# gisbi-kim/navtech-radar-slam

Measured on AMD Instinct MI355X. Metric: sc_loop_queries_per_sec_vs_10k_scan_db, higher is better.
Workload: dtype f16 filter + f64 exact

## Files before the change

navtech-radar-slam_amd/csrc/sc_api.cpp:

```cpp
#include <cmath>
#include <cstdio>
#include <cstdlib>
#include <cstring>
#include <mutex>
#include <new>
#include <string>
#include <vector>

#include "rsx_common.h"
#include "sc_kernels.h"
#include "sc_plan.h"
#include "sc_kdtree.h"
#include "loopverify.h"
#include "radarsc.h"
#include "voxelgrid.h"

namespace rsx {
std::string &last_error() {
  static thread_local std::string e;
  return e;
}
}

using namespace rsx;
// ... 1530 lines not shown
int rsx_sc_merge_topk(const rsx_sc_hit *parts, int32_t nparts, int32_t nq, int32_t k, rsx_sc_hit *out) try {
  if (!parts || !out || nparts < 1 || nq < 1 || k < 1) return fail(RSX_ERR_BAD_ARG, "bad arg");
  for (int q = 0; q < nq; q++) {
    rsx_sc_hit *o = out + (size_t)q * k;
    int count = 0;
    for (int p = 0; p < nparts; p++)
      for (int i = 0; i < k; i++) {
        const rsx_sc_hit &r = parts[((size_t)p * nq + q) * k + i];
        if (!(r.dist < 10000000)) continue;
        int pos = count < k ? count : k;
        while (pos > 0 && ((r.dist < o[pos - 1].dist) || (r.dist == o[pos - 1].dist && r.index < o[pos - 1].index))) pos--;
        if (pos >= k) continue;
        int last = count < k ? count : k - 1;
        for (int j = last; j > pos; j--) o[j] = o[j - 1];
        o[pos] = r;
        if (count < k) count++;
      }
    for (int i = count; i < k; i++) {
      o[i].dist = 10000000;
      o[i].index = 0;
      o[i].shift = 0;
    }
  }
  return RSX_OK;
} RSX_CATCH_ALL

int rsx_sc_merge_topk_device(rsx_sc *h, const rsx_sc_hit *d_parts, int32_t nparts, int32_t nq, int32_t k,
                             rsx_sc_hit *d_out, void *stream) try {
  if (!h || !d_parts || !d_out || nparts < 1 || nq < 1 || k < 1 || k > RSX_SC_MAX_TOPK) return fail(RSX_ERR_BAD_ARG, "bad arg");
  std::lock_guard<std::mutex> lk(h->mu);
  RSX_TRY(set_device(h));
  hipStream_t s;
  RSX_TRY(use_stream(h, stream, &s));
  return launch_merge(d_parts, nparts, nq, k, d_out, s);
} RSX_CATCH_ALL

int rsx_sc_profile_enable(rsx_sc *h, int on) try {
  if (!h) return fail(RSX_ERR_BAD_ARG, "null handle");
  std::lock_guard<std::mutex> lk(h->mu);
  RSX_TRY(own_stream(h));
  if (on && !h->prof.ev) {
    h->prof.ev.reset(new (std::nothrow) Event[2 * PairProfiler::kMax]);
    if (!h->prof.ev) return fail(RSX_ERR_OOM, "host alloc");
    for (int i = 0; i < 2 * PairProfiler::kMax; i++) RSX_HIP(h->prof.ev[i].create(true));
  }
  if (on) {
    RSX_TRY(h->stats.reserve(kStatBytes, h->stream, false));
    RSX_HIP(hipMemsetAsync(h->stats.p, 0, kStatBytes, h->stream));
    RSX_HIP(hipStreamSynchronize(h->stream));
  }
  h->prof.on = on != 0;
  h->prof.used = 0;
  return RSX_OK;
} RSX_CATCH_ALL

int rsx_sc_profile_read_rescoring(rsx_sc *h, rsx_sc_rescoring_stats *out) try {
  if (!h || !out || out->struct_size < offsetof(rsx_sc_rescoring_stats, candidates)) return fail(RSX_ERR_BAD_ARG, "null arg / struct_size not set");
  int64_t out6[8];
  int64_t *const out5 = out6;
  int64_t *candidates = out5, *exact_evals = out5 + 1, *queries_rescored = out5 + 2;
  struct Publish {
    rsx_sc_rescoring_stats *o;
    const int64_t *v;
    ~Publish() {
      int64_t *dst = &o->candidates;
      const size_t n = (o->struct_size - offsetof(rsx_sc_rescoring_stats, candidates)) / sizeof(int64_t);
      for (size_t i = 0; i < n && i < 8; i++) dst[i] = v[i];
    }
  } publish{out, out6};
  std::lock_guard<std::mutex> lk(h->mu);
  RSX_TRY(set_device(h));
  for (int i = 0; i < 8; i++) out6[i] = 0;
  if (!h->stats.p) return RSX_OK;
  RSX_HIP(hipDeviceSynchronize());
  unsigned long long v[RESCORE_STAT_WORDS] = {0};
  {
    std::vector<unsigned long long> all((size_t)RESCORE_STAT_COPIES * RESCORE_STAT_WORDS);
    RSX_HIP(hipMemcpy(all.data(), h->stats.p, kStatBytes, hipMemcpyDeviceToHost));
    RSX_HIP(hipMemset(h->stats.p, 0, kStatBytes));
    for (int c = 0; c < RESCORE_STAT_COPIES; c++)
      for (int i = 0; i < RESCORE_STAT_WORDS; i++) v[i] += all[(size_t)c * RESCORE_STAT_WORDS + i];
  }
  if (rsx::exp_env("RSX_RESCORE_PROF") && v[1])
    fprintf(stderr, "[sc_rescore prof] per query (cycles): start loads %.0f  round filter + touch %.0f  pick %.0f  phaseB %.0f  align %.0f  entry wait %.0f  total %.0f\n",
            (double)v[4] / v[1], (double)v[5] / v[1], (double)v[6] / v[1], (double)v[7] / v[1], (double)v[8] / v[1], (double)v[9] / v[1],
            (double)v[10] / v[1]);
  *candidates = (int64_t)v[0];
  *exact_evals = v[2] ? (int64_t)v[2] : (int64_t)v[0];
  *queries_rescored = (int64_t)v[1];
  out5[3] = (int64_t)v[3];
  out5[4] = (int64_t)v[11];
  out6[5] = v[12] ? (int64_t)v[12] : 7 * *exact_evals;
  out6[6] = (int64_t)v[15];
  out6[7] = (int64_t)v[16];
  return RSX_OK;
} RSX_CATCH_ALL

int rsx_sc_profile_read(rsx_sc *h, int64_t *launches, double *total_ms) try {
  if (!h || !launches || !total_ms) return fail(RSX_ERR_BAD_ARG, "null arg");
  std::lock_guard<std::mutex> lk(h->mu);
  RSX_TRY(set_device(h));
  *launches = 0;
  *total_ms = 0.0;
  for (int i = 0; i < h->prof.used; i++) {
    RSX_HIP(hipEventSynchronize(h->prof.ev[2 * i + 1]));
    float ms = 0.f;
    RSX_HIP(hipEventElapsedTime(&ms, h->prof.ev[2 * i], h->prof.ev[2 * i + 1]));
    *total_ms += ms;
    (*launches)++;
  }
  h->prof.used = 0;
  return RSX_OK;
} RSX_CATCH_ALL

int rsx_sc_hit_to_loop(rsx_sc *h, const rsx_sc_hit *hit, int32_t *loop_id, float *yaw) try {
  if (!h || !hit) return fail(RSX_ERR_BAD_ARG, "null arg");
  std::lock_guard<std::mutex> lk(h->mu);
  if (loop_id) *loop_id = (hit->dist < h->p.dist_thres) ? hit->index : -1;
  if (yaw) *yaw = yaw_from_shift(hit->shift);
  return RSX_OK;
} RSX_CATCH_ALL

}
```

navtech-radar-slam_amd/csrc/sc_exact_dev.h:

```cpp
#pragma once
#include <hip/hip_runtime.h>

#include <cmath>
#include <cstdint>

#include "sc_kernels.h"
#include "sc_entry_dev.h"

namespace rsx {
namespace sc {
namespace {

constexpr double kBig = 10000000.0;

constexpr int ENT_VKEY_A = 0, ENT_VKEY_B = 1152, ENT_SIM = 0, ENT_MISC = 3360;
constexpr int ENT_SIZE = 3408;

__device__ __forceinline__ bool hit_before(double ad, int ai, double bd, int bi) {
  return (ad < bd) || (ad == bd && ai < bi);
}

struct EntryRegs {
  float4 ecol[5];
  double v, n2;
};
__device__ __forceinline__ void load_entry(const DbView &db, int64_t slot, int lane, EntryRegs &r) {
  const int cl = lane < NS ? lane : 0;
  r.v = db.vkey[slot * NS + cl];
  const float4 *src = reinterpret_cast<const float4 *>(db.desc + slot * DS + cl * NR);
#pragma unroll
  for (int i = 0; i < 5; i++) r.ecol[i] = src[i];
  r.n2 = db.norm[slot * NS + cl];
}

struct Touch {
  int d0 = 0, d1 = 0, d2 = 0;
};
__device__ __forceinline__ void touch_entry(const DbView &db, int64_t slot, int lane, Touch &t) {
  const int cl = lane < NS ? lane : 0;
  const float *pd = db.desc + slot * DS + cl * NR;
  const double *pk = db.vkey + slot * NS + cl, *pn = db.norm + slot * NS + cl;
  asm volatile("global_load_dword %0, %3, off\n\tglobal_load_dword %1, %4, off\n\tglobal_load_dword %2, %5, off"
               : "+v"(t.d0), "+v"(t.d1), "+v"(t.d2)
               : "v"(pd), "v"(pk), "v"(pn)
               : "memory");
}
__device__ __forceinline__ void touch_keep(Touch &t) { asm volatile("" : "+v"(t.d0), "+v"(t.d1), "+v"(t.d2)); }
__device__ __forceinline__ void touch_wait(Touch &t) {
  asm volatile("s_waitcnt vmcnt(0)" : "+v"(t.d0), "+v"(t.d1), "+v"(t.d2)::"memory");
}

template <int SO = dev::SO_SSE2>
__device__ __forceinline__ int align_exact(const double *v1, char *wsm, int lane, double ev) {
  const int kk = lane < NS ? lane : NS - 1;
  double *vka = reinterpret_cast<double *>(wsm + ENT_VKEY_A);
  double *vkb = reinterpret_cast<double *>(wsm + ENT_VKEY_B);
  if (lane < NS) {
    vka[lane] = ev;
    vka[lane + NS] = ev;
    vkb[lane + 1] = ev;
    vkb[lane + NS + 1] = ev;
  }
  wave::lds_fence();
  double acc[4] = {0.0, 0.0, 0.0, 0.0};
  const int eoff = (kk & 1) ? (ENT_VKEY_B + (NS + 1 - kk) * 8) : (ENT_VKEY_A + (NS - kk) * 8);
  const double2 *v2 = reinterpret_cast<const double2 *>(wsm + eoff);
  const double2 *v1p = reinterpret_cast<const double2 *>(v1);
#pragma unroll 1
  for (int c0 = 0; c0 < NS / 2; c0 += 6) {
#pragma unroll
    for (int cc = 0; cc < 6; cc++) {
      const double2 x = v1p[c0 + cc], y = v2[c0 + cc];
      const double d0 = x.x - y.x;
      const double dd0 = d0 * d0;
      acc[2 * (cc & 1)] = acc[2 * (cc & 1)] + dd0;
      const double d1 = x.y - y.y;
      const double dd1 = d1 * d1;
      acc[2 * (cc & 1) + 1] = acc[2 * (cc & 1) + 1] + dd1;
    }
  }
  double nrm = sqrt((acc[0] + acc[2]) + (acc[1] + acc[3]));
  if constexpr (SO != dev::SO_SSE2) {
    const double *v1d = v1, *v2d = reinterpret_cast<const double *>(wsm + eoff);
    auto d = [&](int c) { return v1d[c] - v2d[c]; };
    nrm = sqrt(dev::redux_prod<SO, NS>(d, d));
  }
  const bool ok = (lane < NS) && (nrm < kBig);
  double m = ok ? nrm : INFINITY;
  m = wave::butterfly(m, [](double a, double b) { return fmin(a, b); });
  const unsigned long long bal = __ballot(ok && nrm == m);
  wave::lds_fence();
  return bal ? (__ffsll((long long)bal) - 1) : 0;
}

__device__ __forceinline__ void topk_insert(double &ld, int &li, int &ls, int lane, int k, double dist, int idx,
                                            int shift) {
  const bool before = (lane < k) && hit_before(ld, li, dist, idx);
  const int pos = __popcll(__ballot(before));
  if (pos < k) {
    double ud = __shfl_up(ld, 1);
    int ui = __shfl_up(li, 1), us = __shfl_up(ls, 1);
    if (lane > pos) {
      ld = ud; li = ui; ls = us;
    } else if (lane == pos) {
      ld = dist; li = idx; ls = shift;
    }
  }
}

__device__ __forceinline__ void topk_insert_dpp(double &ld, int &li, int &ls, int lane, int k, double dist, int idx, int shift) {
  const bool before = (lane < k) && hit_before(ld, li, dist, idx);
  const int pos = __popcll(__ballot(before));
  if (pos < k) {
    const double ud = wave::dpp<0x138>(ld);
    const int ui = wave::dpp<0x138>(li), us = wave::dpp<0x138>(ls);
    if (lane > pos) {
      ld = ud; li = ui; ls = us;
    } else if (lane == pos) {
      ld = dist; li = idx; ls = shift;
    }
  }
}

struct WaveLds {
  static constexpr int OFF_QF32 = 0;
  static constexpr int OFF_QN1 = DS * 4;
  static constexpr int OFF_QV1 = OFF_QN1 + 512;
  static constexpr int OFF_ENT = OFF_QV1 + 512;
  static constexpr int SIZE = OFF_ENT + ENT_SIZE;
};

template <int SO = dev::SO_SSE2>
__device__ __forceinline__ void phase_b32(const char *smem, char *wsm, int lane, const EntryRegs &er, int ks, unsigned tmask,
                                          double &bd_out, int &bk_out) {
  const int cl = lane < NS ? lane : 0;
  const double *qn1 = reinterpret_cast<const double *>(smem + WaveLds::OFF_QN1);
  wave::lds_fence();
  double e[NR];
#pragma unroll
  for (int i = 0; i < 5; i++) {
    const float4 v = er.ecol[i];
    e[4 * i + 0] = v.x; e[4 * i + 1] = v.y; e[4 * i + 2] = v.z; e[4 * i + 3] = v.w;
  }
  const double n2 = er.n2;
  double *simp = reinterpret_cast<double *>(wsm + ENT_SIM);
  int *misc = reinterpret_cast<int *>(wsm + ENT_MISC);
#pragma unroll
  for (int t = 0; t < 7; t++) {
    if (!((tmask >> t) & 1u)) continue;
    int k = ks + t - 3;
    k += (k < 0) ? NS : 0;
    k -= (k >= NS) ? NS : 0;
    int c = cl + k;
    c -= (c >= NS) ? NS : 0;
    const float4 *qp = reinterpret_cast<const float4 *>(smem + WaveLds::OFF_QF32 + c * (NR * 4));
    double da[4] = {0.0, 0.0, 0.0, 0.0};
#pragma unroll
    for (int i = 0; i < 5; i++) {
      const float4 q4 = qp[i];
      da[0] = fma((double)q4.x, e[4 * i + 0], da[0]);
      da[1] = fma((double)q4.y, e[4 * i + 1], da[1]);
      da[2] = fma((double)q4.z, e[4 * i + 2], da[2]);
      da[3] = fma((double)q4.w, e[4 * i + 3], da[3]);
    }
    double dot = (da[0] + da[2]) + (da[1] + da[3]);
    if constexpr (SO != dev::SO_SSE2) {
      const float *qf = reinterpret_cast<const float *>(qp);
      dot = dev::redux_prod<SO, NR>([&](int r) { return (double)qf[r]; }, [&](int r) { return e[r]; });
    }
    const double n1 = qn1[c];
    const bool valid = (lane < NS) && !((n1 == 0.0) | (n2 == 0.0));
    const double s = dot / (n1 * n2);
    if (lane < NS) simp[t * NS + c] = valid ? s : 0.0;
    const int ne = __popcll(__ballot(valid));
    if (lane == 0) misc[t] = ne;
  }
  wave::lds_fence();
  const int tt = lane & 7;
  double bd = INFINITY;
  int bk = 0x7fffffff;
  if (lane < 8 && tt < 7 && ((tmask >> tt) & 1u)) {
    const double2 *sp = reinterpret_cast<const double2 *>(wsm + ENT_SIM + tt * (NS * 8));
    double s = 0.0;
#pragma unroll 1
    for (int c0 = 0; c0 < NS / 2; c0 += 6) {
#pragma unroll
      for (int cc = 0; cc < 6; cc++) {
        const double2 v = sp[c0 + cc];
        s = s + v.x;
        s = s + v.y;
      }
    }
    const int ne = misc[tt];
    const double d = 1.0 - s / (double)ne;
    int k = ks + tt - 3;
    k += (k < 0) ? NS : 0;
    k -= (k >= NS) ? NS : 0;
    if (d < kBig) {
      bd = d;
      bk = k;
    }
  }
#pragma unroll
  for (int off = 1; off <= 4; off <<= 1) {
    const double od = __shfl_xor(bd, off);
    const int ok = __shfl_xor(bk, off);
    if (hit_before(od, ok, bd, bk)) {
      bd = od;
      bk = ok;
    }
  }
  bd = __shfl(bd, 0);
  bk = __shfl(bk, 0);
  if (bd == INFINITY) {
    bd = kBig;
    bk = 0;
  }
  bd_out = bd;
  bk_out = bk;
}

}
}
}
```

navtech-radar-slam_amd/csrc/sc_filter.hip:

```cpp
#include <hip/hip_runtime.h>

#include <cmath>
#include <cstdint>
#include <cstdlib>
#include <type_traits>
#include <utility>

#include "rsx_common.h"
#include "sc_kernels.h"
#include "sc_entry_dev.h"

namespace rsx {
namespace sc {

namespace {

typedef _Float16 half8 __attribute__((ext_vector_type(8)));
typedef float floatx16 __attribute__((ext_vector_type(16)));
typedef unsigned frag4 __attribute__((ext_vector_type(4)));
typedef unsigned long long u64;

#define AS1 __attribute__((address_space(1)))
#define AS3 __attribute__((address_space(3)))

// ... 255 lines not shown
    const int64_t n = tile * 32 + col;
    const bool n_ok = tile_ok && n < a.n_items;
    const int nphase = (q1 - q0 + F_QPP - 1) / F_QPP;

    {
      const int nqs = (q1 - q0 < F_QPP) ? (q1 - q0) : F_QPP;
      stage_queries(a.qimg + (int64_t)q0 * FILTER_QIMG_BYTES, smem, nqs * FILTER_QIMG_BYTES, wave, lane);
    }

    half8 B[F_STEPS];
    {
      const uint4 *src = a.hnT + ((tile_ok ? tile : 0) * F_STEPS) * 64 + lane;
#pragma unroll
      for (int s = 0; s < F_STEPS; s++) {
        const uint4 v = src[s * 64];
        B[s] = *reinterpret_cast<const half8 *>(&v);
      }
#pragma unroll
      for (int s = F_B_VGPR; s < F_STEPS; s++) asm volatile("" : "+a"(B[s]));
    }
    const u64 m2 = n_ok ? a.cmask[n] : 0ull;
    const unsigned m2lo = (unsigned)m2, m2hi = (unsigned)(m2 >> 32) & 0x0fffffffu;

    asm volatile("s_waitcnt vmcnt(0)" ::: "memory");
    __syncthreads();

    floatx16 acc0, acc1, p0;
    frag4 first[F_DEPTH];
    int prev_q = -1;
    u64 prev_mask = 0;
    auto fin = [&](const Epi &ep) {
      float best = epi_end(ep);
      if ((prev_mask | m2) & kNonFinite) best = -INFINITY;
      if (n_ok && hh == 0) a.lb[(int64_t)prev_q * a.ld_lb + n] = lb_pack(best);
    };
    for (int p = 0; p < nphase; p++) {
      const int qp = q0 + p * F_QPP;
      if (p + 1 < nphase) {
        const int qn = qp + F_QPP;
        const int nqs = (q1 - qn < F_QPP) ? (q1 - qn) : F_QPP;
        stage_queries(a.qimg + (int64_t)qn * FILTER_QIMG_BYTES, smem + ((p + 1) & 1) * F_PHASE_BYTES,
                      nqs * FILTER_QIMG_BYTES, wave, lane);
      }
      const int nq_here = (q1 - qp < F_QPP) ? (q1 - qp) : F_QPP;
      if (tile_ok) {
        const unsigned phase_lds = lds_base + (unsigned)((p & 1) * F_PHASE_BYTES + aoff);
        first_prologue(first, phase_lds);
        for (int qq = 0; qq < nq_here; qq++) {
          const unsigned ap_lds = phase_lds + (unsigned)(qq * FILTER_QIMG_BYTES);
          const unsigned next_lds = (qq + 1 < nq_here) ? ap_lds + FILTER_QIMG_BYTES : ap_lds;
          const u64 cur_mask = *reinterpret_cast<const u64 *>(smem + (p & 1) * F_PHASE_BYTES + qq * FILTER_QIMG_BYTES + QIMG_MASK_OFF);
          if (prev_q < 0) filter_stage<true, false>(ap_lds, next_lds, first, B, acc0, acc1, p0, prev_mask, m2lo, m2hi, hh, fin);
          else filter_stage<true, true>(ap_lds, next_lds, first, B, acc0, acc1, p0, prev_mask, m2lo, m2hi, hh, fin);
          prev_q = qp + qq;
          prev_mask = cur_mask;
        }
      }
      asm volatile("s_waitcnt vmcnt(0)" ::: "memory");
      __syncthreads();
    }
    if (prev_q >= 0) filter_stage<false, true>(0u, 0u, first, B, acc0, acc1, p0, prev_mask, m2lo, m2hi, hh, fin);
  }
}

constexpr int H_BINS = RESCORE_BINS;
constexpr int SEL_U = 5;

struct Elig {
  int64_t idx_base, idx_stride, n_eligible;
  const int64_t *q_elig;
};
__device__ __forceinline__ int64_t n_elig_items(const Elig &el, int q, int64_t n_items) {
  int64_t lim = el.n_eligible;
  if (el.q_elig) {
    const int64_t v = el.q_elig[q];
    lim = v < lim ? v : lim;
  }
  if (lim <= el.idx_base) return 0;
  const int64_t c = (lim - el.idx_base + el.idx_stride - 1) / el.idx_stride;
  return c < n_items ? c : n_items;
}


__global__ __launch_bounds__(256) void sc_select_kernel(const lb_t *__restrict__ lb, int64_t ld, int64_t n_items_all,
                                                        Elig el, int32_t first_target,
                                                        RescoreEntry *__restrict__ slist,
                                                        int32_t *__restrict__ sl_cnt, float *__restrict__ thr) {
  __shared__ int hist[H_BINS];
  __shared__ int wsum[4];
  __shared__ int s_bcap;
  __shared__ int s_total;
  const int q = blockIdx.x;
  const int lane = threadIdx.x & 63, wave = threadIdx.x >> 6;
  const lb_t *row = lb + (int64_t)q * ld;
  const int64_t n_items = n_elig_items(el, q, n_items_all);
  for (int i = threadIdx.x; i < H_BINS; i += 256) hist[i] = 0;
  if (threadIdx.x == 0) s_total = 0;
  __syncthreads();
  typedef _Float16 half8 __attribute__((ext_vector_type(8)));
  const uint4 *row8 = reinterpret_cast<const uint4 *>(row);
  const int64_t n8 = n_items >> 3;
  const bool one_piece = n8 <= 256 * SEL_U;
  uint4 keep[SEL_U];
  auto load_piece = [&](int64_t c0, uint4 (&x)[SEL_U]) {
#pragma unroll
    for (int u = 0; u < SEL_U; u++) {
      const int64_t j = c0 + u * 256 + threadIdx.x;
      x[u] = j < n8 ? row8[j] : uint4{0x7c007c00u, 0x7c007c00u, 0x7c007c00u, 0x7c007c00u};
    }
  };
  auto walk_piece = [&](int64_t c0, const uint4 (&x)[SEL_U], auto &&f) {
#pragma unroll
    for (int u = 0; u < SEL_U; u++) {
      const int64_t i = (c0 + u * 256 + threadIdx.x) << 3;
      const half8 h = __builtin_bit_cast(half8, x[u]);
#pragma unroll
      for (int e = 0; e < 8; e++) f((float)h[e], i + e);
    }
  };
  auto for_row = [&](bool first, auto &&f) {
    if (one_piece) {
      if (first) load_piece(0, keep);
      walk_piece(0, keep, f);
    } else {
      for (int64_t c0 = 0; c0 < n8; c0 += 256 * SEL_U) {
        uint4 x[SEL_U];
        load_piece(c0, x);
        walk_piece(c0, x, f);
      }
    }
    const int64_t i = (n8 << 3) + threadIdx.x;
    if (i < n_items) f((float)row[i], i);
  };
  for_row(true, [&](float d, int64_t) {
    if (d != INFINITY) atomicAdd(&hist[lb_bin(d)], 1);
  });
  __syncthreads();
  int v[8];
  int run = 0;
#pragma unroll
  for (int i = 0; i < 8; i++) {
    run += hist[threadIdx.x * 8 + i];
    v[i] = run;
  }
  const int incl = (int)wave::incl_add_u32((unsigned)run);
  if (lane == 63) wsum[wave] = incl;
  __syncthreads();
  int base = incl - run;
  for (int w = 0; w < wave; w++) base += wsum[w];
  __syncthreads();
#pragma unroll
  for (int i = 0; i < 8; i++) hist[threadIdx.x * 8 + i] = base + v[i];
  __syncthreads();
  auto first_reaching = [&](int target) {
    int lo = 0, hi = H_BINS;
    while (lo < hi) {
      const int mid = (lo + hi) >> 1;
      if (hist[mid] >= target) hi = mid;
      else lo = mid + 1;
    }
    return lo;
  };
  if (threadIdx.x == 0) s_bcap = first_reaching(RESCORE_SHORTLIST_CAP + 1) - 1;
  __syncthreads();
  const int b_cap = s_bcap;
  if (threadIdx.x < RESCORE_NUM_THR) {
    int b = b_cap;
    if (threadIdx.x < RESCORE_NUM_THR - 1) {
      b = first_reaching(first_target << threadIdx.x);
      if (b > H_BINS - 1) b = H_BINS - 1;
      if (b > b_cap) b = b_cap;
    }
    thr[(int64_t)q * RESCORE_THR_STRIDE + threadIdx.x] = lb_bin_edge(b);
    reinterpret_cast<int32_t *>(thr)[(int64_t)q * RESCORE_THR_STRIDE + RESCORE_NUM_THR + threadIdx.x] = b >= 0 ? hist[b] : 0;
  }
  int b_head = first_reaching(RESCORE_HEAD);
  if (b_head > b_cap) b_head = b_cap;
  if (threadIdx.x == 0) {
    int32_t *hd = reinterpret_cast<int32_t *>(thr) + (int64_t)q * RESCORE_THR_STRIDE;
    hd[RESCORE_THR_HEAD_BIN] = b_head;
    hd[RESCORE_THR_HEAD_END] = b_head >= 0 ? hist[b_head] : 0;
  }
  RescoreEntry *out = slist + (int64_t)q * RESCORE_SHORTLIST_CAP;
  __shared__ int fill[H_BINS];
  for (int i = threadIdx.x; i < H_BINS; i += 256) fill[i] = i ? hist[i - 1] : 0;
  __syncthreads();
  if (b_head >= 0) {
    for_row(false, [&](float d, int64_t i) {
      if (d == INFINITY) return;
      const int b = lb_bin(d);
      if (b > b_head) return;
      RescoreEntry e;
      e.lb = d;
      e.slot = (int32_t)i;
      out[atomicAdd(&fill[b], 1)] = e;
    });
  }
  if (threadIdx.x == 0) s_total = b_cap >= 0 ? hist[b_cap] : 0;
  __syncthreads();
  if (threadIdx.x == 0) sl_cnt[q] = s_total;
}

__global__ __launch_bounds__(1024) void sc_filter_plan_kernel(Elig el, int32_t nq, int64_t n_items, int32_t qgroup,
                                                              int32_t *__restrict__ tb_qmin, int64_t *__restrict__ tb_cum) {
  __shared__ long long sh[1024];
  const int64_t ntb = (((n_items + 31) >> 5) + 3) >> 2;
  const int t = threadIdx.x;
  long long running = 0;
  for (int64_t base = 0; base < ntb; base += 1024) {
    const int64_t tb = base + t;
    long long items = 0;
    if (tb < ntb) {
      const int64_t g0 = el.idx_base + tb * 128 * el.idx_stride;
      int lo = 0, hi = nq;
      while (lo < hi) {
        const int mid = (lo + hi) >> 1;
        int64_t lim = el.n_eligible;
        if (el.q_elig) {
          const int64_t v = el.q_elig[mid];
          lim = v < lim ? v : lim;
        }
        if (lim > g0) hi = mid;
        else lo = mid + 1;
      }
      tb_qmin[tb] = lo / qgroup;
      items = (nq + qgroup - 1) / qgroup - lo / qgroup;
    }
    sh[t] = items;
    __syncthreads();
    for (int d = 1; d < 1024; d <<= 1) {
      const long long v = t >= d ? sh[t - d] : 0;
      __syncthreads();
      sh[t] += v;
      __syncthreads();
    }
    if (tb < ntb) tb_cum[tb] = running + sh[t] - items;
    running += sh[1023];
    __syncthreads();
  }
  if (t == 0) tb_cum[ntb] = running;
}

}

double filter_eps() {
  static const double eps = [] {
    const char *e = rsx::exp_env("RSX_SC_FILTER_EPS");
    const double v = e ? atof(e) : 0.0;
    return v > 1.25e-3 ? v : 1.25e-3;
  }();
  return eps;
}

size_t filter_qimg_bytes(int32_t nq) { return (size_t)nq * FILTER_QIMG_BYTES + 1024; }

int launch_db_images(const float *desc, const double *norm, int64_t first, int64_t count, void *hnT, void *hnR,
                     uint64_t *cmask, hipStream_t s) {
  if (count <= 0) return RSX_OK;
  hipLaunchKernelGGL(sc_img_db_kernel, dim3((unsigned)((count + 3) / 4)), dim3(256), 0, s, desc, norm, first, count,
                     static_cast<uint4 *>(hnT), static_cast<uint4 *>(hnR), reinterpret_cast<u64 *>(cmask));
  RSX_HIP(hipGetLastError());
  return RSX_OK;
}

int launch_query_images(const float *desc, const double *norm, int32_t nq, void *qimg, hipStream_t s) {
  if (nq <= 0) return RSX_OK;
  hipLaunchKernelGGL(sc_img_query_kernel, dim3((unsigned)((nq + 3) / 4)), dim3(256), 0, s, desc, norm, nq,
                     static_cast<char *>(qimg));
  RSX_HIP(hipGetLastError());
  return RSX_OK;
}

const char *filter_kernel_name() { return "sc_filter_kernel"; }

size_t filter_plan_bytes(int64_t n_items) {
  const int64_t ntb = (((n_items + 31) / 32) + 3) / 4;
  return (size_t)(ntb + 1) * sizeof(int64_t) + (size_t)ntb * sizeof(int32_t) + 64;
}

int launch_filter_plan(const DbView &db, const FilterPlanInput &plan, int32_t nq, int64_t n_items, int32_t qgroup,
                       void *plan_ws, const int32_t **tb_qmin, const int64_t **tb_cum, hipStream_t s) {
  const int64_t ntb = (((n_items + 31) / 32) + 3) / 4;
  int64_t *cum = static_cast<int64_t *>(plan_ws);
  int32_t *qmin = reinterpret_cast<int32_t *>(cum + ntb + 1);
  const Elig el{db.idx_base, db.idx_stride, plan.n_eligible < 0 ? INT64_MAX : plan.n_eligible, plan.q_elig};
  hipLaunchKernelGGL(sc_filter_plan_kernel, dim3(1), dim3(1024), 0, s, el, nq, n_items, qgroup, qmin, cum);
  RSX_HIP(hipGetLastError());
  *tb_qmin = qmin;
  *tb_cum = cum;
  return RSX_OK;
}

int launch_filter(const DbView &db, const void *qimg, int32_t nq, int64_t n_items, lb_t *lb, int64_t ld_lb,
                  const FilterPlanInput *plan, void *plan_ws, hipStream_t s) {
  if (nq <= 0 || n_items <= 0) return RSX_OK;
  static int n_cu = 0;
  const int lds = 2 * F_PHASE_BYTES;
  if (!n_cu) {
    RSX_HIP(hipFuncSetAttribute(reinterpret_cast<const void *>(&sc_filter_kernel),
                                hipFuncAttributeMaxDynamicSharedMemorySize, lds));
    int dev = 0, cu = 0;
    RSX_HIP(hipGetDevice(&dev));
    RSX_HIP(hipDeviceGetAttribute(&cu, hipDeviceAttributeMultiprocessorCount, dev));
    n_cu = cu > 0 ? cu : 256;
  }
  FilterArgs a;
  a.hnT = static_cast<const uint4 *>(db.hnT);
  a.cmask = reinterpret_cast<const u64 *>(db.cmask);
  a.qimg = static_cast<const char *>(qimg);
  a.n_items = n_items;
  a.nq = nq;
  a.lb = lb;
  a.ld_lb = ld_lb;
  const int64_t ntiles = (n_items + 31) / 32;
  const int64_t total = ((ntiles + 3) / 4) * (int64_t)nq;
  int64_t per = (total + n_cu - 1) / n_cu;
  if (per < 16) per = 16;
  const int64_t nblk = (total + per - 1) / per;
  a.per_block = per;
  a.tb_qmin = nullptr;
  a.tb_cum = nullptr;
  unsigned grid = (unsigned)nblk;
  if (plan && plan_ws) {
    RSX_TRY(launch_filter_plan(db, *plan, nq, n_items, 1, plan_ws, &a.tb_qmin, &a.tb_cum, s));
    grid = (unsigned)n_cu;
  }
  hipLaunchKernelGGL(sc_filter_kernel, dim3(grid), dim3(256), lds, s, a);
  RSX_HIP(hipGetLastError());
  return RSX_OK;
}

int launch_select(const DbView &db, const lb_t *lb, int64_t ld_lb, int64_t n_items, int32_t nq, int64_t n_eligible,
                  const int64_t *q_elig, int32_t first_target, RescoreEntry *slist, int32_t *sl_cnt, float *thr,
                  hipStream_t s) {
  if (nq <= 0) return RSX_OK;
  if (first_target < 1 || first_target > 128) return fail(RSX_ERR_INTERNAL, "bad first_target");
  const Elig el{db.idx_base, db.idx_stride, n_eligible < 0 ? INT64_MAX : n_eligible, q_elig};
  hipLaunchKernelGGL(sc_select_kernel, dim3(nq), dim3(256), 0, s, lb, ld_lb, n_items, el, first_target, slist, sl_cnt, thr);
  RSX_HIP(hipGetLastError());
  return RSX_OK;
}

}
}
```

navtech-radar-slam_amd/csrc/sc_kernels.hip:

```cpp
#include <hip/hip_runtime.h>

#include <cmath>
#include <cstdint>
#include <cstdio>
#include <cstdlib>

#include "rsx_common.h"
#include "sc_kernels.h"
#include "sc_entry_dev.h"
#include "sc_exact_dev.h"

namespace rsx {
namespace sc {

namespace {

using dev::wave_keys;


template <int SO>
__global__ __launch_bounds__(256) void sc_keys_kernel(const float *__restrict__ desc, int64_t n,
                                                      double *__restrict__ vkey, double *__restrict__ norm,
                                                      float *__restrict__ rkey) {
  const int lane = threadIdx.x & 63;
// ... 865 lines not shown
  if (a.partial) {
    hipLaunchKernelGGL(sc_merge_kernel, dim3(q.nq), dim3(64), 0, s, (const rsx_sc_hit *)d_partial, 1,
                       (int64_t)0, (int64_t)a.nslots * k, a.nslots * k, k, d_topk);
    RSX_HIP(hipGetLastError());
  }
  return RSX_OK;
}



#ifndef RW_OCC
#define RW_OCC 3
#endif
template <int SO>
__global__ __launch_bounds__(64, RW_OCC) void sc_rescore_wave_kernel(RescoreArgs a) {
  extern __shared__ __attribute__((aligned(16))) char smem[];
  if (a.stats) a.stats += (blockIdx.x % RESCORE_STAT_COPIES) * RESCORE_STAT_WORDS;
  const int lane = threadIdx.x;
  const int qi = blockIdx.x;
  char *wsm = smem + WaveLds::OFF_ENT;

  const int sl_cnt = a.sl_cnt[qi];
  const float *thr = a.thr + (int64_t)qi * RESCORE_THR_STRIDE;
  const int32_t *rcnt = reinterpret_cast<const int32_t *>(thr) + RESCORE_NUM_THR;
  const float t_cap = thr[RESCORE_NUM_THR - 1];
  const WindowSurvivor *sv = a.surv ? a.surv + (int64_t)qi * WINDOW_LIST_STRIDE : nullptr;
  WindowListHeader hdr;
  hdr.count = 0;
  hdr.tau_ub = INFINITY;
  hdr.n_cand = 0;
  hdr.n_prev = 0;
  WindowSurvivor first;
  first.lo = INFINITY;
  first.slot = 0;
  first.ks = -1;
  first.pos = 0;
  if (sv) {
    hdr = *reinterpret_cast<const WindowListHeader *>(sv);
    first = sv[1 + lane];
  }
  {
    const float4 *src = reinterpret_cast<const float4 *>(a.q.desc + (int64_t)qi * DS);
    float4 *dst = reinterpret_cast<float4 *>(smem + WaveLds::OFF_QF32);
    float4 x[5];
#pragma unroll
    for (int i = 0; i < 5; i++) x[i] = (lane + 64 * i < DS / 4) ? src[lane + 64 * i] : float4{0.f, 0.f, 0.f, 0.f};
    const double kn = lane < NS ? a.q.norm[(int64_t)qi * NS + lane] : 0.0;
    const double kv = lane < NS ? a.q.vkey[(int64_t)qi * NS + lane] : 0.0;
#pragma unroll
    for (int i = 0; i < 5; i++)
      if (lane + 64 * i < DS / 4) dst[lane + 64 * i] = x[i];
    if (lane < NS) {
      reinterpret_cast<double *>(smem + WaveLds::OFF_QN1)[lane] = kn;
      reinterpret_cast<double *>(smem + WaveLds::OFF_QV1)[lane] = kv;
    }
    wave::lds_fence();
  }

  int64_t n_elig = a.n_eligible;
  if (a.q_elig) {
    const int64_t e = a.q_elig[qi];
    n_elig = e < n_elig ? e : n_elig;
  }
  int64_t n_rows = 0;
  if (n_elig > a.db.idx_base) {
    n_rows = (n_elig - a.db.idx_base + a.db.idx_stride - 1) / a.db.idx_stride;
    n_rows = n_rows < a.n_items ? n_rows : a.n_items;
  }

  double ld = INFINITY;
  int li = 0x7fffffff, ls = 0;
  double tau_init = INFINITY;
  if (a.tau_src) {
    const double d = a.tau_src[(int64_t)qi * a.k + (a.k - 1)].dist;
    if (d < kBig) tau_init = d;
  }
  if (a.seed && lane < a.k) {
    const rsx_sc_hit h = a.seed[(int64_t)qi * a.k + lane];
    if (h.dist < kBig) {
      ld = h.dist; li = h.index; ls = h.shift;
    }
  }
  auto kth_of = [&](double list) {
    const double t = __shfl(list, a.k - 1);
    return t < tau_init ? t : tau_init;
  };
  double tau = kth_of(ld);
  unsigned n_exact = 0, n_looked = 0, n_aligned = 0, n_shifts = 0, n_tail = 0;
  unsigned n_listed = 0, n_windowed = 0;
  bool walked_tail = false;

#ifdef RSX_EXPERIMENTS
  const bool timing = a.stats != nullptr;
#else
  constexpr bool timing = false;
#endif
  long long tacc[6] = {0, 0, 0, 0, 0, 0};
  long long t_mark = timing ? clock64() : 0;
  const long long t_begin = t_mark;
  auto lap = [&](int slot_) {
    if (!timing) return;
    const long long t = clock64();
    tacc[slot_] += t - t_mark;
    t_mark = t;
  };
  auto eval = [&](int64_t slot, int ksm, const EntryRegs &er) {
    if (timing) {
      lap(2);
      asm volatile("s_waitcnt vmcnt(0)" ::: "memory");
      lap(5);
    }
    int ks = ksm;
    unsigned tmask = 0x7fu;
    if (ksm >= 0) {
      ks = ksm & 63;
      const unsigned m7 = ((unsigned)ksm >> 8) & 0x7fu;
      if (m7) tmask = m7;
    }
    if (ks < 0) {
      ks = align_exact<SO>(reinterpret_cast<const double *>(smem + WaveLds::OFF_QV1), wsm, lane, er.v);
      n_aligned++;
      lap(4);
    }
    double bd;
    int bk;
    phase_b32<SO>(smem, wsm, lane, er, ks, tmask, bd, bk);
    if (timing) {
      asm volatile("" : "+v"(bd));
      lap(3);
    }
    n_exact++;
    n_shifts += (unsigned)__builtin_popcount(tmask);
    const int64_t gidx = a.db.idx_base + slot * a.db.idx_stride;
    if (gidx < n_elig && bd < kBig) {
      topk_insert(ld, li, ls, lane, a.k, bd, (int)gidx, bk);
      tau = kth_of(ld);
    }
  };

  const RescoreEntry *sl = a.slist + (int64_t)qi * RESCORE_SHORTLIST_CAP;
  const int r_end = a.round_end < RESCORE_NUM_THR ? a.round_end : RESCORE_NUM_THR;
  auto upto = [&](int r) {
    if (r <= 0) return 0;
    const int c = rcnt[r - 1];
    return c < sl_cnt ? c : sl_cnt;
  };
  const int i0 = upto(a.round_begin), i1 = upto(r_end);
  if (timing) {
    int keep = i0 + i1;
    asm volatile("" : "+s"(keep));
    asm volatile("s_waitcnt vmcnt(0)" ::: "memory");
    lap(0);
  }
  bool done = false;

  int pos_next = i0;
  if (sv && i0 < WINDOW_P && i0 < i1) {
    const int pw = i1 < WINDOW_P ? i1 : WINDOW_P;
    const int n_list = hdr.count < WINDOW_P ? hdr.count : WINDOW_P;
    const double tau_ub = (double)hdr.tau_ub;
    if (i0 == 0) {
      n_listed = (unsigned)hdr.n_cand;
      n_windowed = (unsigned)hdr.n_prev;
    }
    for (int base = 0; base < n_list; base += 64) {
      WindowSurvivor e = first;
      if (base > 0 && base + lane < n_list) e = sv[1 + base + lane];
      const double t_now = tau < tau_ub ? tau : tau_ub;
      const bool mine = base + lane < n_list && e.pos >= i0 && e.pos < pw && !((double)e.lo > t_now);
      float mylo = mine ? e.lo : INFINITY;
      const int32_t myslot = e.slot;
      const int myks = e.ks;
      unsigned long long todo = __ballot(mine);
      if (!todo) continue;
      {
        Touch tch;
        for (; todo; todo &= todo - 1) touch_entry(a.db, __shfl(myslot, __ffsll((long long)todo) - 1), lane, tch);
        touch_wait(tch);
      }
      lap(1);
      auto pick = [&](int32_t &slot, int &ks) -> float {
        const float wm = wave::min_f32(mylo);
        if (wm == INFINITY) return wm;
        const int src = __ffsll((long long)__ballot(mylo == wm)) - 1;
        slot = __shfl(myslot, src);
        ks = __shfl(myks, src);
        if (lane == src) mylo = INFINITY;
        return wm;
      };
      EntryRegs cur, nxt;
      int32_t cur_slot = 0, nxt_slot = 0;
      int cur_ks = -1, nxt_ks = -1;
      float cur_lo = pick(cur_slot, cur_ks);
      if (cur_lo < INFINITY) load_entry(a.db, cur_slot, lane, cur);
      while (cur_lo < INFINITY) {
        const double t_eff = tau < tau_ub ? tau : tau_ub;
        if ((double)cur_lo > t_eff) break;
        const float nxt_lo = pick(nxt_slot, nxt_ks);
        if (nxt_lo < INFINITY && !((double)nxt_lo > t_eff)) load_entry(a.db, nxt_slot, lane, nxt);
        eval(cur_slot, cur_ks, cur);
        cur_lo = nxt_lo;
        cur_slot = nxt_slot;
        cur_ks = nxt_ks;
        cur = nxt;
      }
    }
    pos_next = pw > i0 ? pw : i0;
  }

  const int head_bin = rcnt[RESCORE_THR_HEAD_BIN - RESCORE_NUM_THR], head_end = rcnt[RESCORE_THR_HEAD_END - RESCORE_NUM_THR];
  const int i1h = i1 < head_end ? i1 : head_end;
  for (int base = pos_next; base < i1h && !done; base += 64) {
    const int n_here = (i1h - base < 64) ? (i1h - base) : 64;
    RescoreEntry mine;
    mine.lb = INFINITY;
    mine.slot = 0;
    if (lane < n_here) mine = sl[base + lane];
    for (int i = 0; i < n_here; i++) {
      const float lb = __shfl(mine.lb, i);
      const int32_t slot = __shfl(mine.slot, i);
      if ((double)lb_bin_lo(lb_bin(lb)) - a.eps > tau) {
        done = true;
        break;
      }
      if ((double)lb - a.eps > tau) continue;
      const int64_t gidx = a.db.idx_base + (int64_t)slot * a.db.idx_stride;
      if (!(gidx < n_elig)) continue;
      EntryRegs er;
      load_entry(a.db, slot, lane, er);
      n_looked++;
      eval(slot, -1, er);
    }
  }

  if (!done && i1 > head_end) {
    const lb_t *row = a.lb + (int64_t)qi * a.ld_lb;
    const int b_to = lb_edge_bin(thr[r_end - 1]);
    int b = head_bin;
    if (a.round_begin > 0) {
      const int b0 = lb_edge_bin(thr[(a.round_begin < RESCORE_NUM_THR ? a.round_begin : RESCORE_NUM_THR) - 1]);
      b = b0 > b ? b0 : b;
    }
    bool take = false;
    walked_tail = b < b_to;
    while (!done && walked_tail) {
      int next = RESCORE_BINS;
      constexpr int U = 4;
      for (int64_t pos = 0; pos < n_rows && !done; pos += 64 * U) {
        float d[U];
#pragma unroll
        for (int u = 0; u < U; u++) {
          const int64_t i = pos + 64 * u + lane;
          d[u] = (i < n_rows) ? (float)row[i] : INFINITY;
        }
#pragma unroll
        for (int u = 0; u < U; u++) {
          const int bin = (d[u] != INFINITY) ? lb_bin(d[u]) : RESCORE_BINS;
          if (bin > b && bin < next) next = bin;
          unsigned long long bal = __ballot(take && bin == b);
          while (bal && !done) {
            const int l = __ffsll((long long)bal) - 1;
            bal &= bal - 1;
            if ((double)lb_bin_lo(b) - a.eps > tau) {
              done = true;
              break;
            }
            const float dl = __shfl(d[u], l);
            if ((double)dl - a.eps > tau) continue;
            const int64_t slot = pos + 64 * u + l;
            EntryRegs er;
            load_entry(a.db, slot, lane, er);
            n_looked++;
            n_tail++;
            eval(slot, -1, er);
          }
        }
      }
      if (done) break;
      next = wave::butterfly(next, [](int x, int o) { return o < x ? o : x; });
      if (next > b_to) break;
      b = next;
      take = true;
      if ((double)lb_bin_lo(b) - a.eps > tau) done = true;
    }
  }

  if (!done && a.round_end > RESCORE_NUM_THR && t_cap < INFINITY && !((double)t_cap - a.eps > tau)) {
    const lb_t *row = a.lb + (int64_t)qi * a.ld_lb;
// ... 89 lines not shown
```

Before: 3.345 million.

## Overlap first entry load with touch prefetches and rank window survivors upfront

Survivors in each window batch are now ranked once, replacing the repeated wave-min pick. The first entry is loaded asynchronously while the remaining entries are touched, and the wait uses a vmcnt that lets the first entry's data arrive before the touches finish. The touch wait is deferred until after the first evaluation, so cache warming overlaps with compute. Several shuffles in the reductions and top-k insert are swapped for DPP and readlane forms, and an optional select-kernel profiler is added behind a compile flag. This adds inline asm that relies on vmcnt ordering, and the rank loop costs O(n) readlanes per survivor batch.

```diff
diff --git a/navtech-radar-slam_amd/csrc/sc_api.cpp b/navtech-radar-slam_amd/csrc/sc_api.cpp
--- a/navtech-radar-slam_amd/csrc/sc_api.cpp
+++ b/navtech-radar-slam_amd/csrc/sc_api.cpp
@@ -1636,7 +1636,7 @@
       for (int i = 0; i < RESCORE_STAT_WORDS; i++) v[i] += all[(size_t)c * RESCORE_STAT_WORDS + i];
   }
   if (rsx::exp_env("RSX_RESCORE_PROF") && v[1])
-    fprintf(stderr, "[sc_rescore prof] per query (cycles): start loads %.0f  round filter + touch %.0f  pick %.0f  phaseB %.0f  align %.0f  entry wait %.0f  total %.0f\n",
+    fprintf(stderr, "[sc_rescore prof] per query (cycles): start loads %.0f  round filter + rank + touch %.0f  between evaluations %.0f  phaseB %.0f  align %.0f  entry wait %.0f  total %.0f\n",
             (double)v[4] / v[1], (double)v[5] / v[1], (double)v[6] / v[1], (double)v[7] / v[1], (double)v[8] / v[1], (double)v[9] / v[1],
             (double)v[10] / v[1]);
   *candidates = (int64_t)v[0];
diff --git a/navtech-radar-slam_amd/csrc/sc_exact_dev.h b/navtech-radar-slam_amd/csrc/sc_exact_dev.h
--- a/navtech-radar-slam_amd/csrc/sc_exact_dev.h
+++ b/navtech-radar-slam_amd/csrc/sc_exact_dev.h
@@ -49,6 +49,47 @@
 __device__ __forceinline__ void touch_wait(Touch &t) {
   asm volatile("s_waitcnt vmcnt(0)" : "+v"(t.d0), "+v"(t.d1), "+v"(t.d2)::"memory");
 }
+
+typedef float f32x4 __attribute__((ext_vector_type(4)));
+struct EntryAsync {
+  f32x4 c0, c1, c2, c3, c4;
+  double v, n2;
+};
+__device__ __forceinline__ void load_entry_async(const DbView &db, int64_t slot, int lane, EntryAsync &r) {
+  const int cl = lane < NS ? lane : 0;
+  const float *pd = db.desc + slot * DS + cl * NR;
+  const double *pk = db.vkey + slot * NS + cl, *pn = db.norm + slot * NS + cl;
+  asm volatile("global_load_dwordx2 %0, %7, off\n\t"
+               "global_load_dwordx4 %1, %8, off\n\t"
+               "global_load_dwordx4 %2, %8, off offset:16\n\t"
+               "global_load_dwordx4 %3, %8, off offset:32\n\t"
+               "global_load_dwordx4 %4, %8, off offset:48\n\t"
+               "global_load_dwordx4 %5, %8, off offset:64\n\t"
+               "global_load_dwordx2 %6, %9, off"
+               : "=&v"(r.v), "=&v"(r.c0), "=&v"(r.c1), "=&v"(r.c2), "=&v"(r.c3), "=&v"(r.c4), "=&v"(r.n2)
+               : "v"(pk), "v"(pd), "v"(pn)
+               : "memory");
+}
+#define RSX_VMCNT_CASE(n) \
+  case n: asm volatile("s_waitcnt vmcnt(" #n ")" ::: "memory"); break;
+__device__ __forceinline__ void entry_wait(EntryAsync &r, int n_touches, EntryRegs &out) {
+  switch (n_touches < 20 ? 3 * n_touches : 60) {
+    RSX_VMCNT_CASE(0) RSX_VMCNT_CASE(3) RSX_VMCNT_CASE(6) RSX_VMCNT_CASE(9) RSX_VMCNT_CASE(12) RSX_VMCNT_CASE(15)
+    RSX_VMCNT_CASE(18) RSX_VMCNT_CASE(21) RSX_VMCNT_CASE(24) RSX_VMCNT_CASE(27) RSX_VMCNT_CASE(30) RSX_VMCNT_CASE(33)
+    RSX_VMCNT_CASE(36) RSX_VMCNT_CASE(39) RSX_VMCNT_CASE(42) RSX_VMCNT_CASE(45) RSX_VMCNT_CASE(48) RSX_VMCNT_CASE(51)
+    RSX_VMCNT_CASE(54) RSX_VMCNT_CASE(57)
+    default: asm volatile("s_waitcnt vmcnt(60)" ::: "memory"); break;
+  }
+  asm volatile("" : "+v"(r.v), "+v"(r.c0), "+v"(r.c1), "+v"(r.c2), "+v"(r.c3), "+v"(r.c4), "+v"(r.n2));
+  out.v = r.v;
+  out.n2 = r.n2;
+  out.ecol[0] = float4{r.c0.x, r.c0.y, r.c0.z, r.c0.w};
+  out.ecol[1] = float4{r.c1.x, r.c1.y, r.c1.z, r.c1.w};
+  out.ecol[2] = float4{r.c2.x, r.c2.y, r.c2.z, r.c2.w};
+  out.ecol[3] = float4{r.c3.x, r.c3.y, r.c3.z, r.c3.w};
+  out.ecol[4] = float4{r.c4.x, r.c4.y, r.c4.z, r.c4.w};
+}
+#undef RSX_VMCNT_CASE
 
 template <int SO = dev::SO_SSE2>
 __device__ __forceinline__ int align_exact(const double *v1, char *wsm, int lane, double ev) {
@@ -87,7 +128,10 @@
   }
   const bool ok = (lane < NS) && (nrm < kBig);
   double m = ok ? nrm : INFINITY;
-  m = wave::butterfly(m, [](double a, double b) { return fmin(a, b); });
+  {
+    auto mn = [](double a, double b) { return fmin(a, b); };
+    m = wave::rows_pair(wave::row_reduce(m, mn), mn);
+  }
   const unsigned long long bal = __ballot(ok && nrm == m);
   wave::lds_fence();
   return bal ? (__ffsll((long long)bal) - 1) : 0;
@@ -201,17 +245,17 @@
       bk = k;
     }
   }
-#pragma unroll
-  for (int off = 1; off <= 4; off <<= 1) {
-    const double od = __shfl_xor(bd, off);
-    const int ok = __shfl_xor(bk, off);
+  auto take = [&](double od, int ok) {
     if (hit_before(od, ok, bd, bk)) {
       bd = od;
       bk = ok;
     }
-  }
-  bd = __shfl(bd, 0);
-  bk = __shfl(bk, 0);
+  };
+  take(wave::dpp<0xB1>(bd), wave::dpp<0xB1>(bk));
+  take(wave::dpp<0x4E>(bd), wave::dpp<0x4E>(bk));
+  take(wave::dpp<0x141>(bd), wave::dpp<0x141>(bk));
+  bd = wave::readlane(bd, 0);
+  bk = wave::readlane(bk, 0);
   if (bd == INFINITY) {
     bd = kBig;
     bk = 0;
diff --git a/navtech-radar-slam_amd/csrc/sc_filter.hip b/navtech-radar-slam_amd/csrc/sc_filter.hip
--- a/navtech-radar-slam_amd/csrc/sc_filter.hip
+++ b/navtech-radar-slam_amd/csrc/sc_filter.hip
@@ -361,10 +361,41 @@
 }
 
 
+#ifdef RSX_SELECT_PROF
+constexpr bool kSelProf = true, kSelLaps = RSX_SELECT_PROF == 1;
+#else
+constexpr bool kSelProf = false, kSelLaps = false;
+#endif
+enum SelProfRegion {
+  SP_LOAD = 0,
+  SP_HIST,
+  SP_SCAN,
+  SP_COMPACT,
+  SP_TOTAL,
+  SP_COUNT,
+  SEL_PROF_WORDS
+};
+constexpr int SEL_PROF_COPIES = 64;
+
 __global__ __launch_bounds__(256) void sc_select_kernel(const lb_t *__restrict__ lb, int64_t ld, int64_t n_items_all,
                                                         Elig el, int32_t first_target,
                                                         RescoreEntry *__restrict__ slist,
-                                                        int32_t *__restrict__ sl_cnt, float *__restrict__ thr) {
+                                                        int32_t *__restrict__ sl_cnt, float *__restrict__ thr,
+                                                        unsigned long long *prof, int cap_mode) {
+  long long t_mark = 0, t_begin = 0, tacc[SP_TOTAL] = {0, 0, 0, 0};
+  if constexpr (kSelLaps) t_begin = t_mark = clock64();
+  auto lap = [&](int region) {
+    if constexpr (kSelLaps) {
+      asm volatile("s_waitcnt vmcnt(0) lgkmcnt(0)" ::: "memory");
+      const long long t = clock64();
+      tacc[region] += t - t_mark;
+      t_mark = t;
+    }
+  };
+  int cap_bin = H_BINS;
+  if constexpr (kSelProf) {
+    if (cap_mode) cap_bin = lb_edge_bin(thr[(int64_t)blockIdx.x * RESCORE_THR_STRIDE + RESCORE_NUM_THR - 1]) + 1;
+  }
   __shared__ int hist[H_BINS];
   __shared__ int wsum[4];
   __shared__ int s_bcap;
@@ -399,7 +430,10 @@
   };
   auto for_row = [&](bool first, auto &&f) {
     if (one_piece) {
-      if (first) load_piece(0, keep);
+      if (first) {
+        load_piece(0, keep);
+        lap(SP_LOAD);
+      }
       walk_piece(0, keep, f);
     } else {
       for (int64_t c0 = 0; c0 < n8; c0 += 256 * SEL_U) {
@@ -412,9 +446,13 @@
     if (i < n_items) f((float)row[i], i);
   };
   for_row(true, [&](float d, int64_t) {
+    if constexpr (kSelProf) {
+      if (lb_bin(d) > cap_bin) return;
+    }
     if (d != INFINITY) atomicAdd(&hist[lb_bin(d)], 1);
   });
   __syncthreads();
+  lap(SP_HIST);
   int v[8];
   int run = 0;
 #pragma unroll
@@ -464,6 +502,7 @@
   __shared__ int fill[H_BINS];
   for (int i = threadIdx.x; i < H_BINS; i += 256) fill[i] = i ? hist[i - 1] : 0;
   __syncthreads();
+  lap(SP_SCAN);
   if (b_head >= 0) {
     for_row(false, [&](float d, int64_t i) {
       if (d == INFINITY) return;
@@ -478,6 +517,16 @@
   if (threadIdx.x == 0) s_total = b_cap >= 0 ? hist[b_cap] : 0;
   __syncthreads();
   if (threadIdx.x == 0) sl_cnt[q] = s_total;
+  if constexpr (kSelLaps) {
+    lap(SP_COMPACT);
+    if (prof && lane == 0) {
+      unsigned long long *o = prof + (size_t)(q % SEL_PROF_COPIES) * SEL_PROF_WORDS;
+#pragma unroll
+      for (int r = 0; r < SP_TOTAL; r++) atomicAdd(o + r, (unsigned long long)tacc[r]);
+      atomicAdd(o + SP_TOTAL, (unsigned long long)(t_mark - t_begin));
+      atomicAdd(o + SP_COUNT, 1ull);
+    }
+  }
 }
 
 __global__ __launch_bounds__(1024) void sc_filter_plan_kernel(Elig el, int32_t nq, int64_t n_items, int32_t qgroup,
@@ -615,8 +664,34 @@
   if (nq <= 0) return RSX_OK;
   if (first_target < 1 || first_target > 128) return fail(RSX_ERR_INTERNAL, "bad first_target");
   const Elig el{db.idx_base, db.idx_stride, n_eligible < 0 ? INT64_MAX : n_eligible, q_elig};
-  hipLaunchKernelGGL(sc_select_kernel, dim3(nq), dim3(256), 0, s, lb, ld_lb, n_items, el, first_target, slist, sl_cnt, thr);
+#ifndef RSX_SELECT_PROF
+  hipLaunchKernelGGL(sc_select_kernel, dim3(nq), dim3(256), 0, s, lb, ld_lb, n_items, el, first_target, slist, sl_cnt, thr,
+                     static_cast<unsigned long long *>(nullptr), 0);
   RSX_HIP(hipGetLastError());
+#else
+  constexpr size_t kProfWords = (size_t)SEL_PROF_COPIES * SEL_PROF_WORDS;
+  static unsigned long long *d_prof = nullptr;
+  if (!d_prof) RSX_HIP(hipMalloc(reinterpret_cast<void **>(&d_prof), kProfWords * 8));
+  static const bool capped = [] {
+    const char *e = getenv("RSX_SELECT_CAP_ATOMICS");
+    return e && atoi(e) != 0;
+  }();
+  for (int pass = 0; pass < (capped ? 2 : 1); pass++) {
+    RSX_HIP(hipMemsetAsync(d_prof, 0, kProfWords * 8, s));
+    hipLaunchKernelGGL(sc_select_kernel, dim3(nq), dim3(256), 0, s, lb, ld_lb, n_items, el, first_target, slist, sl_cnt, thr, d_prof, pass);
+    RSX_HIP(hipGetLastError());
+    static unsigned long long h[kProfWords];
+    RSX_HIP(hipMemcpyAsync(h, d_prof, kProfWords * 8, hipMemcpyDeviceToHost, s));
+    RSX_HIP(hipStreamSynchronize(s));
+    double v[SEL_PROF_WORDS] = {0};
+    for (int c = 0; c < SEL_PROF_COPIES; c++)
+      for (int i = 0; i < SEL_PROF_WORDS; i++) v[i] += (double)h[(size_t)c * SEL_PROF_WORDS + i];
+    if (v[SP_COUNT] > 0)
+      fprintf(stderr, "[sc_select prof] nq %d%s (cycles per wave, %.0f reported):  load %.0f  histogram %.0f  scan + edges %.0f  compaction %.0f  total %.0f\n",
+              (int)nq, pass ? " capped" : "", v[SP_COUNT], v[SP_LOAD] / v[SP_COUNT], v[SP_HIST] / v[SP_COUNT], v[SP_SCAN] / v[SP_COUNT],
+              v[SP_COMPACT] / v[SP_COUNT], v[SP_TOTAL] / v[SP_COUNT]);
+  }
+#endif
   return RSX_OK;
 }
 
diff --git a/navtech-radar-slam_amd/csrc/sc_kernels.hip b/navtech-radar-slam_amd/csrc/sc_kernels.hip
--- a/navtech-radar-slam_amd/csrc/sc_kernels.hip
+++ b/navtech-radar-slam_amd/csrc/sc_kernels.hip
@@ -971,7 +971,7 @@
     }
   }
   auto kth_of = [&](double list) {
-    const double t = __shfl(list, a.k - 1);
+    const double t = wave::readlane(list, a.k - 1);
     return t < tau_init ? t : tau_init;
   };
   double tau = kth_of(ld);
@@ -1022,7 +1022,7 @@
     n_shifts += (unsigned)__builtin_popcount(tmask);
     const int64_t gidx = a.db.idx_base + slot * a.db.idx_stride;
     if (gidx < n_elig && bd < kBig) {
-      topk_insert(ld, li, ls, lane, a.k, bd, (int)gidx, bk);
+      topk_insert_dpp(ld, li, ls, lane, a.k, bd, (int)gidx, bk);
       tau = kth_of(ld);
     }
   };
@@ -1057,42 +1057,58 @@
       if (base > 0 && base + lane < n_list) e = sv[1 + base + lane];
       const double t_now = tau < tau_ub ? tau : tau_ub;
       const bool mine = base + lane < n_list && e.pos >= i0 && e.pos < pw && !((double)e.lo > t_now);
-      float mylo = mine ? e.lo : INFINITY;
+      const float mylo = mine ? e.lo : INFINITY;
       const int32_t myslot = e.slot;
       const int myks = e.ks;
-      unsigned long long todo = __ballot(mine);
+      const unsigned long long todo = __ballot(mine);
       if (!todo) continue;
-      {
-        Touch tch;
-        for (; todo; todo &= todo - 1) touch_entry(a.db, __shfl(myslot, __ffsll((long long)todo) - 1), lane, tch);
-        touch_wait(tch);
-      }
-      lap(1);
-      auto pick = [&](int32_t &slot, int &ks) -> float {
-        const float wm = wave::min_f32(mylo);
-        if (wm == INFINITY) return wm;
-        const int src = __ffsll((long long)__ballot(mylo == wm)) - 1;
-        slot = __shfl(myslot, src);
-        ks = __shfl(myks, src);
-        if (lane == src) mylo = INFINITY;
-        return wm;
+      const int n_mine = __popcll(todo);
+      int myrank = 0;
+      for (unsigned long long m = todo; m; m &= m - 1) {
+        const int j = __ffsll((long long)m) - 1;
+        const float x = wave::readlane(mylo, j);
+        myrank += (x < mylo || (x == mylo && j < lane)) ? 1 : 0;
+      }
+      auto ranked = [&](int i, int32_t &slot, int &ks) -> float {
+        if (i >= n_mine) return INFINITY;
+        const unsigned long long at = __ballot(mine && myrank == i);
+        if (!at) return INFINITY;
+        const int src = __ffsll((long long)at) - 1;
+        slot = wave::readlane(myslot, src);
+        ks = wave::readlane(myks, src);
+        return wave::readlane(mylo, src);
       };
       EntryRegs cur, nxt;
       int32_t cur_slot = 0, nxt_slot = 0;
       int cur_ks = -1, nxt_ks = -1;
-      float cur_lo = pick(cur_slot, cur_ks);
-      if (cur_lo < INFINITY) load_entry(a.db, cur_slot, lane, cur);
+      int rank_next = 0;
+      float cur_lo = ranked(rank_next++, cur_slot, cur_ks);
+      Touch tch;
+      bool touching = cur_lo < INFINITY;
+      if (touching) {
+        EntryAsync ea;
+        load_entry_async(a.db, cur_slot, lane, ea);
+        const unsigned long long rest = todo & ~__ballot(mine && myrank == 0);
+        for (unsigned long long m = rest; m; m &= m - 1) touch_entry(a.db, wave::readlane(myslot, __ffsll((long long)m) - 1), lane, tch);
+        entry_wait(ea, __popcll(rest), cur);
+      }
+      lap(1);
       while (cur_lo < INFINITY) {
         const double t_eff = tau < tau_ub ? tau : tau_ub;
         if ((double)cur_lo > t_eff) break;
-        const float nxt_lo = pick(nxt_slot, nxt_ks);
+        const float nxt_lo = ranked(rank_next++, nxt_slot, nxt_ks);
         if (nxt_lo < INFINITY && !((double)nxt_lo > t_eff)) load_entry(a.db, nxt_slot, lane, nxt);
         eval(cur_slot, cur_ks, cur);
+        if (touching) {
+          touch_wait(tch);
+          touching = false;
+        }
         cur_lo = nxt_lo;
         cur_slot = nxt_slot;
         cur_ks = nxt_ks;
         cur = nxt;
       }
+      if (touching) touch_wait(tch);
     }
     pos_next = pw > i0 ? pw : i0;
   }
```

Result: faster. 3.391 million, median of 6 (+1.4%).
